# davidepi/glaze

Measured on AMD Instinct MI355X. Metric: Msamples/s + achieved HBM GB/s, Sponza 1080p, 1/2/4/8xMI355X, higher is better.
Workload: dtype f32; 1 GPU; Sponza-class synthetic atrium (262267 tris, 26 materials, 27 textures) as a .glaze V1 file (2853389 bytes) through parse, 1920x1080, path tracer depth 8, 143 steps = 17.9 spp; materials=26, textures=27, scene=Sponza-class synthetic atrium, width=1920, height=1080, depth=8, triangles=262267

## Files before the change

glaze_amd/csrc/device/path_state.h:

```cpp
#pragma once
#include <hip/hip_runtime.h>

#include "device/intersect.h"
#include "device/math.h"
#include "device/trace_wave.h"
#include "kernels.h"

namespace glz {
using namespace dev;

constexpr uint32_t kQueueShards = 8;
constexpr uint32_t kCounterStride = 32;
constexpr uint32_t kFlagUpdate = 1u;
constexpr uint32_t kFlagShadow = 2u;

struct PixelId {
  uint32_t x, y;
  bool active;
};
__device__ __forceinline__ PixelId pixel_of(const TileMap& m, uint32_t lid) {
  const uint32_t lane = lid & 63u, sub = (lid >> 6) & 63u, ltile = lid >> 12;
  const uint32_t gtile = ltile * m.world + m.rank;
  const uint32_t tx = gtile % m.tiles_x, ty = gtile / m.tiles_x;
  PixelId p;
// ... 53 lines not shown
      direction = mk3(rd.x, rd.y, rd.z);
    }
    tmin = 0.0001f;
    tmax = INFINITY;
    return true;
  }
};
__device__ __forceinline__ float4 pack_hit(const HitRecord& h) { return make_float4(h.leaf == 0xFFFFFFFFu ? INFINITY : h.t, h.u, h.v, __uint_as_float(h.leaf)); }
struct ClosestSink {
  const LaunchArgs& A;
  __device__ __forceinline__ void store(uint32_t lid, const HitRecord& h) { A.st.hit[lid] = pack_hit(h); }
};

__device__ __forceinline__ float update_mark(uint32_t ordinal) { return -(float)(ordinal < (1u << 24) ? ordinal : (1u << 24)); }
__device__ __forceinline__ void accumulate_retired(const LaunchArgs& A, uint32_t lid, vec3 c, bool add, float mark, float4 cum) {
  if (add) A.st.cumulative[lid] = make_float4(cum.x + c.x, cum.y + c.y, cum.z + c.z, mark);
  else A.st.cumulative[lid].w = mark;
}
__device__ __forceinline__ void accumulate_shaded(const LaunchArgs& A, uint32_t lid, vec3 c, bool add, bool update, float mark) {
  if (!update) return;
  if (add) {
    const float4 cum = A.st.cumulative[lid];
    A.st.cumulative[lid] = make_float4(cum.x + c.x, cum.y + c.y, cum.z + c.z, mark);
  } else {
    A.st.cumulative[lid].w = mark;
  }
}

__device__ __forceinline__ uint32_t queue_capacity(uint32_t n_local_pixels) {
  const uint32_t blocks = (n_local_pixels + kBlock - 1) / kBlock;
  return ((blocks + kQueueShards - 1) / kQueueShards) * kBlock;
}
__device__ __forceinline__ uint32_t queue_slot(uint32_t* counters, uint32_t n_local_pixels, bool push) {
  const unsigned long long m = __ballot(push);
  uint32_t slot = 0;
  if (push) {
    const uint32_t shard = ((blockIdx.x * blockDim.x + threadIdx.x) / kBlock) % kQueueShards;
    const int lane = threadIdx.x & 63;
    const int leader = __ffsll((long long)m) - 1;
    uint32_t base = 0;
    if (lane == leader) base = atomicAdd(counters + shard * kCounterStride, (uint32_t)__popcll(m));
    base = __shfl(base, leader);
    slot = shard * queue_capacity(n_local_pixels) + base + (uint32_t)__popcll(m & ((1ull << lane) - 1ull));
  }
  return slot;
}

struct ShadowSource {
  const LaunchArgs& A;
  const uint32_t* start;
  uint32_t cap;
  uint32_t lid;
  float4 contrib;
  __device__ __forceinline__ bool load(uint32_t i, vec3& o, vec3& d, float& tmin, float& tmax) {
    uint32_t shard = 0;
#pragma unroll
    for (uint32_t k = 1; k < kQueueShards; ++k) shard += i >= start[k] ? 1u : 0u;
    const uint32_t q = shard * cap + (i - start[shard]);
    const float4 so = A.st.sh_o[q], sd = A.st.sh_d[q];
    contrib = A.st.contrib[q];
    lid = __float_as_uint(sd.w);
    o = mk3(so.x, so.y, so.z);
    d = mk3(sd.x, sd.y, sd.z);
    tmin = 0.001f;
    tmax = so.w;
    return true;
  }
};
struct ShadowSink {
  const LaunchArgs& A;
  ShadowSource& src;
  __device__ __forceinline__ void store(uint32_t, const HitRecord& h) {
    const bool occluded = h.leaf != 0xFFFFFFFFu;
    const vec3 c = mk3(src.contrib.x, src.contrib.y, src.contrib.z);
    if (occluded) A.st.cumulative[src.lid].w = A.shadow_mark;
    else accumulate_retired(A, src.lid, c, true, A.shadow_mark, A.st.cumulative[src.lid]);
  }
};
__device__ __forceinline__ void clear_next_queue_set(const LaunchArgs& A) {
  if (blockIdx.x == 0 && threadIdx.x < kQueueShards) A.st.queue_count[A.shade_set * kQueueSetWords + threadIdx.x * kCounterStride] = 0;
}
}
```

glaze_amd/csrc/device/tuning.h:

```cpp
#pragma once
#ifndef GLZ_TRACE_WAVES
#define GLZ_TRACE_WAVES 6
#endif
#ifndef GLZ_TRACE_SPLIT_NUM
#define GLZ_TRACE_SPLIT_NUM 8
#endif
#ifndef GLZ_TRACE_SPLIT_DEN
#define GLZ_TRACE_SPLIT_DEN 10
#endif
#ifndef GLZ_ANY_FAR_FIRST
#define GLZ_ANY_FAR_FIRST 1
#endif
#ifndef GLZ_COUNT_ANY_FAR_FIRST
#define GLZ_COUNT_ANY_FAR_FIRST 0
#endif
#ifndef GLZ_TRACE_PREFETCH
#define GLZ_TRACE_PREFETCH 0
#endif
#ifndef GLZ_TRACE_TL_WAVES
#define GLZ_TRACE_TL_WAVES 4
#endif
#ifndef GLZ_SHADE_WAVES
#define GLZ_SHADE_WAVES 4
#endif
#ifndef GLZ_PATH_WAVES
#define GLZ_PATH_WAVES 4
#endif
#ifndef GLZ_TRACE8_WAVES
#define GLZ_TRACE8_WAVES 4
#endif
#ifndef GLZ_TRACE8_STACK
#define GLZ_TRACE8_STACK 28
#endif
#ifndef GLZ_TRACE8_PREFETCH
#define GLZ_TRACE8_PREFETCH 1
#endif
#ifndef GLZ_REFILL
#define GLZ_REFILL 10
#endif
#ifndef GLZ_REFILL_ANY
#define GLZ_REFILL_ANY GLZ_REFILL
#endif
#ifndef GLZ_LEAF_QUORUM_ANY
#define GLZ_LEAF_QUORUM_ANY 30
#endif
#ifndef GLZ_TL_REFILL
#define GLZ_TL_REFILL 16
#endif
#ifndef GLZ_LEAF_QUORUM
#define GLZ_LEAF_QUORUM 24
#endif
#ifndef GLZ_ALPHA_QUORUM
#define GLZ_ALPHA_QUORUM 12
#endif
#ifndef GLZ_TL_LEAF_QUORUM
#define GLZ_TL_LEAF_QUORUM 32
#endif
#ifndef GLZ_PATH_PREFETCH
#define GLZ_PATH_PREFETCH 1
#endif
```

glaze_amd/csrc/kernels.h:

```cpp
#pragma once
#include <hip/hip_runtime.h>
#include <stdint.h>

#include <vector>

#include "device/types.h"
#include "glaze_abi.h"
#include "device_buffer.h"
#include "reproject.h"

namespace glz {

hipError_t launch_derivatives(hipStream_t st, const float4* vertices, const uint32_t* indices, uint32_t n_tris, float4* out);

struct HierarchyInputs {
  const float4* vertices;
  const uint32_t* indices;
  const RTInstance* instances;
  const uint32_t* inst_base;
  uint32_t n_instances;
  const TransformPair* transforms;
  const RTMaterial* materials;
  uint32_t n_world;
  int builder;
  float pair_area_ratio;
  const float4* given_lo = nullptr;
  const float4* given_hi = nullptr;
  bool emit_quads = false;
  bool emit_wide8 = false;
};
constexpr int kBvhBuilderLbvh = 0, kBvhBuilderPloc = 1, kBvhBuilderSah = 2, kBvhBuilderAuto = 3, kBvhBuilderSahHost = 4;
void build_sah_host(uint32_t n, const float4* lo, const float4* hi, int2* children, int* parent);
struct HierarchyOutputs {
  DeviceBuffer<BvhNode4> nodes;
  DeviceBuffer<BvhNode8> nodes8;
  uint32_t depth8;
  BvhGrid grid;
  BvhTri* tris;
  DeviceBuffer<BvhQuad> quads;
  uint32_t depth;
  float sah;
  float bounds_lo[3], bounds_hi[3];
};
hipError_t build_hierarchy(hipStream_t st, const HierarchyInputs& in, HierarchyOutputs& out);
hipError_t launch_top_table(hipStream_t st, const BvhNode4* nodes, uint32_t n_nodes, BvhNode4* top);
hipError_t launch_shade_records(hipStream_t st, uint32_t n, const BvhTri* tris, const RTInstance* instances, const uint32_t* indices,
                                const float4* vertices, const float4* derivatives, const uint32_t* xf_identity, float4* out);
struct InstanceBoxItem {
  uint32_t transform, mesh, first, count;
};
hipError_t launch_instance_boxes(hipStream_t st, uint32_t n_items, const InstanceBoxItem* items, const float4* points, const TransformPair* xf,
                                 double* partial, uint32_t n_instances, const uint32_t* item_first, const float4* mesh_lo, const float4* mesh_hi,
                                 float4* box_lo, float4* box_hi);
hipError_t launch_alpha_records(hipStream_t st, uint32_t n, const float4* shade_tris, const RTMaterial* materials, const TexDesc* tex_desc, float4* out);

hipError_t launch_refit_leaves(hipStream_t st, const float4* vertices, const uint32_t* indices, const RTInstance* instances, const TransformPair* transforms,
                               uint32_t n_leaves, BvhQuad* quads, BvhTri* tris, float4* leaf_lo, float4* leaf_hi);
struct RefitNodes {
// ... 14 lines not shown

struct TraversalSizes {
  uint64_t n_nodes, n_nodes8, n_leaves, n_instances, grid_lanes, overflow_depth;
};
const char* traversal_offsets_exceeded(const TraversalSizes& sizes);

struct PathState {
  float4* ray_o;
  float4* ray_d;
  float4* imp[4];
  float4* hit;
  float* cone;
  uint32_t* hit_inst;
  float4* sh_o;
  float4* sh_d;
  float4* contrib;
  uint32_t* queue_count;
  float4* cumulative;
  float4* result;
  uint32_t* overflow;
  uint32_t overflow_depth;
  uint32_t* path_cost;
};

struct TileMap {
  uint32_t width, height;
  uint32_t tiles_x, tiles_y;
  uint32_t rank, world;
  uint32_t n_local_tiles;
  uint32_t n_local_pixels;
};

struct CameraConsts {
  float camera2world[16];
  float screen2camera[16];
};

struct TraceCounters {
  unsigned long long closest_rays, shadow_rays, closest_nodes, closest_tris, shadow_nodes, shadow_tris, hits, fresh;
  unsigned long long phase[12];
  unsigned long long shade_tex[4], trace_tex[4];
};

struct LaunchArgs {
  DeviceScene scene;
  PathState st;
  TileMap map;
  FrameData frame;
  CameraConsts cam;
  TraceCounters* counters;
  uint32_t do_closest, do_shadow;
  uint32_t shade_set;
  float shadow_mark;
};
constexpr uint32_t kPathMaxLaunches = 192;
struct PathBatch {
  uint32_t n;
  uint32_t tables_in_lds;
  uint32_t parity;
  uint32_t seed[kPathMaxLaunches];
  float offset[kPathMaxLaunches + 1][2];
  uint32_t base_ordinal;
};
constexpr uint32_t kTraceBlock = 256;
constexpr uint32_t kQueueSetWords = 8 * 32;

uint32_t trace_grid_blocks(uint32_t n_local_pixels, bool counting, bool two_level, bool wide8 = false);
hipError_t launch_trace(hipStream_t st, const LaunchArgs& a, uint32_t blocks, bool wide8 = false);
hipError_t launch_shade(hipStream_t st, const LaunchArgs& a);
uint32_t path_grid_blocks(uint32_t n_local_pixels, const DeviceScene& scene);
uint32_t path_resident_blocks(const DeviceScene& scene);
hipError_t launch_path(hipStream_t st, const LaunchArgs& a, const PathBatch& batch, uint32_t blocks);
hipError_t launch_finalize(hipStream_t st, const TileMap& map, float4* cumulative, float4* result, float exposure, float launches);
hipError_t launch_export(hipStream_t st, const TileMap& map, const float4* tiled, float4* frame, bool zero_first);
hipError_t launch_pack_tiles(hipStream_t st, uint32_t n_chain_pixels, uint32_t n_chains, uint32_t chain, const float4* tiled, float4* packed);
hipError_t launch_tonemap(hipStream_t st, uint32_t n_pixels, const float4* result_frame, const float* thresholds, uchar4* out);

uint32_t first_hit_grid_blocks(uint32_t n_rays);
hipError_t launch_first_hit(hipStream_t st, const LaunchArgs& a, uint32_t blocks, float4* hit, uint32_t* inst);
hipError_t launch_first_hit_attributes(hipStream_t st, const LaunchArgs& a, const float4* hit, const uint32_t* inst, float4* aov0, float4* aov1);
constexpr uint32_t kGuideCountWords = GLZ_GUIDE_MAX_BOUNCES + 2;
struct GuideLists {
  float4* o[2];
  float4* d[2];
  uint32_t* count;
};
uint32_t guide_grid_blocks(uint32_t n_rays, uint32_t first_hit_blocks);
hipError_t launch_guide_chain(hipStream_t st, const LaunchArgs& a, uint32_t blocks, uint32_t max_bounces, uint32_t last_list, float4* hit, uint32_t* inst,
                              const GuideLists& lists, float4* aov0, float4* aov1);
hipError_t launch_guide_scatter(hipStream_t st, uint32_t blocks, const GuideLists& lists, uint32_t list, uint32_t n_pixels, float* origins3, float* dirs3,
                                uint8_t* alive);
hipError_t launch_camera_rays(hipStream_t st, const LaunchArgs& a, float off_x, float off_y, float* origins3, float* dirs3);
hipError_t launch_denoise(hipStream_t st, uint32_t w, uint32_t h, const glz_denoise_params& params, const float4* result, const float4* aov0,
                          const float4* aov1, float4* ping, float4* pong, float4* out, hipEvent_t* marks = nullptr,
                          const glz_despeckle_params* despeckle = nullptr, hipEvent_t* despeckle_marks = nullptr);
hipError_t launch_despeckle(hipStream_t st, uint32_t w, uint32_t h, const glz_despeckle_params& params, float eps_albedo, const float4* result,
                            const float4* aov0, const float4* aov1, float4* ping, float4* out, hipEvent_t* despeckle_marks = nullptr);
hipError_t launch_motion(hipStream_t st, const LaunchArgs& a, const float4* hit, const uint32_t* inst, const float4* prev_o2w, const post::ProjectConstants& prev,
                         float4* motion, const float4* prev_vertices = nullptr, uint32_t first_vertex = 0, uint32_t n_vertices = 0);
hipError_t launch_reproject(hipStream_t st, uint32_t w, uint32_t h, const glz_reproject_params& params, const float4* motion, const float4* prev_color,
                            const float4* prev_aov0, const float4* prev_aov1, float4* out, hipEvent_t* marks = nullptr);
hipError_t launch_project_points(hipStream_t st, const post::ProjectConstants& C, uint32_t w, uint32_t h, const float* points3, uint32_t n, float* out3);

struct SkinArgs {
  const float4* bind;
  const uint2* joints;
  const float4* weights;
  uint32_t n;
  const float4* bones;
  uint32_t n_bones;
  int blend;
};
constexpr uint32_t kSkinLdsBones = 256;
struct MorphArgs {
  const float4* base;
  const uint32_t* counts;
  const uint2* slices;
  const float4* entries;
// ... 57 lines not shown
```

glaze_amd/csrc/kernels_render.hip:

```cpp
#include "device/path_state.h"
#include "device/shade_pixel.h"
#include "device/trace_wave.h"
#include "device/trace_wave_tl.h"
#include "launch_geometry.h"
#include "symbol_readers.h"

namespace glz {
using namespace dev;


constexpr uint32_t kShadeBlock = 256, kShadeWavesPerBlock = kShadeBlock / 64;
#ifdef GLZ_SECTION_TIMES
static __device__ unsigned long long g_shade_sections[16 * 4096];
#endif
__host__ __device__ inline bool shade_tables_fit(const DeviceScene& s) { return SceneTables(s).bytes() <= kShadeLdsTableBytes; }
__host__ __device__ inline bool shade_sky_fits(const DeviceScene& s) { return s.sky_header.marginal_cdf_count > 1u && s.sky_header.marginal_cdf_count <= kSkyLdsFloats; }
template <class T>
__device__ __forceinline__ const T* in_memory(const T* p) { return (const T*)(const __attribute__((address_space(1))) T*)p; }
template <bool COUNT, bool LOD, bool TABLES, bool SKY>
__global__ void __launch_bounds__(kShadeBlock, GLZ_SHADE_WAVES) k_shade(const LaunchArgs A) {
#ifdef GLZ_SECTION_TIMES
  unsigned long long ks[4] = {0, 0, 0, 0}, ks_last = __builtin_amdgcn_s_memtime();
#define GLZ_KS(k) do { const unsigned long long now_ = __builtin_amdgcn_s_memtime(); ks[k] += now_ - ks_last; ks_last = now_; } while (0)
#else
// ... 129 lines not shown
  {
    __syncthreads();
    float4* stage = reinterpret_cast<float4*>(s_pool);
    const uint32_t p = s_perm[threadIdx.x];
    s_bin[p] = staged.mask;
    if (staged.mask & 1u) stage[p] = staged.ro;
    if (staged.mask & 2u) stage[kShadeBlock + p] = staged.rd;
    if (staged.mask & 4u) {
#pragma unroll
      for (int q = 0; q < 4; ++q) stage[(2u + q) * kShadeBlock + p] = staged.im[q];
    }
    __syncthreads();
    const LaunchArgs& A3 = *(const LaunchArgs*)reread_kernarg();
    const uint32_t m = s_bin[threadIdx.x], at = blockIdx.x * kShadeBlock + threadIdx.x;
    if (m & 1u) A3.st.ray_o[at] = stage[threadIdx.x];
    if (m & 2u) A3.st.ray_d[at] = stage[kShadeBlock + threadIdx.x];
    if (m & 4u) {
#pragma unroll
      for (int q = 0; q < 4; ++q) A3.st.imp[q][at] = stage[(2u + q) * kShadeBlock + threadIdx.x];
    }
  }
  if (COUNT) flush_tex_tallies(A.counters->shade_tex, tex_tally);
#ifdef GLZ_SECTION_TIMES
  if (!COUNT) {
    GLZ_KS(3);
    unsigned long long v[10] = {ks[0], ks[1], ks[2], staged.sec[0], staged.sec[1], staged.sec[2], staged.sec[3], staged.sec[4], staged.sec[5], ks[3]};
    const uint32_t w = blockIdx.x * kShadeWavesPerBlock + (threadIdx.x >> 6);
#pragma unroll
    for (int k = 0; k < 10; ++k) {
      unsigned int lo = (unsigned int)v[k], hi = (unsigned int)(v[k] >> 32);
      for (int off = 32; off > 0; off >>= 1) {
        const unsigned int lo2 = __shfl_xor(lo, off), hi2 = __shfl_xor(hi, off);
        const unsigned long long a = ((unsigned long long)hi << 32) | lo, b = ((unsigned long long)hi2 << 32) | lo2;
        if (b > a) { lo = lo2; hi = hi2; }
      }
      if ((threadIdx.x & 63u) == 0u && w < 4096u) g_shade_sections[16u * w + k] += ((unsigned long long)hi << 32) | lo;
    }
    if ((threadIdx.x & 63u) == 0u && w < 4096u) g_shade_sections[16u * w + 15u] += 1ull;
  }
#endif
}

template <bool COUNT, int ALPHA>
__global__ void __launch_bounds__(kBlock, GLZ_TRACE_WAVES) k_trace(const LaunchArgs A) {
  __shared__ int s_stack[kLdsStack * kBlock];
  __shared__ alignas(1024) int s_aux[kAuxPerBlock];
  __shared__ uint4 s_top[kBvhTopNodes * 4];
  static_assert(kBvhTopNodes * 4 <= kBlock, "stage_top copies one 16-byte piece per thread");
  GLZ_WAVE_STAMP(0);
  stage_top(A.scene, s_top);
  int* aux = wave_aux(s_aux, threadIdx.x >> 6);
  int* links = wave_links(s_aux, threadIdx.x >> 6);
  clear_next_queue_set(A);
  unsigned long long tex_tally[4] = {0ull, 0ull, 0ull, 0ull};
  DeviceScene counted_scene;
  if (COUNT) {
    counted_scene = A.scene;
    counted_scene.tex_counter = tex_tally;
  }
  const DeviceScene& TS = COUNT ? counted_scene : A.scene;
  uint32_t split_closest = A.do_closest, split_shadow = A.do_shadow, split_wave_c = wave_index(), split_waves_c = wave_count(), split_wave_s = 0, split_waves_s = 0;
  bool split = false;
  if (!COUNT && A.do_closest && A.do_shadow) {
    const uint32_t* counts0 = A.st.queue_count + (A.shade_set ^ 1u) * kQueueSetWords;
    uint32_t n_sh = 0;
#pragma unroll
    for (uint32_t k = 0; k < kQueueShards; ++k) n_sh += counts0[k * kCounterStride];
    const uint32_t gc = (A.map.n_local_pixels + 63u) / 64u, gs = (n_sh + 63u) / 64u, nw = wave_count();
    if (gc + gs > nw && gs > 0u) {
      split = true;
      uint32_t ws = (uint32_t)(((unsigned long long)nw * gs * GLZ_TRACE_SPLIT_NUM) / ((unsigned long long)gc * GLZ_TRACE_SPLIT_DEN + (unsigned long long)gs * GLZ_TRACE_SPLIT_NUM));
      ws = ws < 1u ? 1u : (ws > nw - 1u ? nw - 1u : ws);
      const uint32_t w = wave_index();
      const uint32_t s_before = (uint32_t)(((unsigned long long)w * ws) / nw), s_after = (uint32_t)(((unsigned long long)(w + 1u) * ws) / nw);
      const bool is_shadow = s_after > s_before;
      split_closest = is_shadow ? 0u : 1u;
      split_shadow = is_shadow ? 1u : 0u;
      split_wave_c = w - s_before;
      split_waves_c = nw - ws;
      split_wave_s = s_before;
      split_waves_s = ws;
    }
  }
  if (split_closest) {
    TraceTally tally;
    ClosestSource src{A, A.frame, tally, 0u};
    ClosestSink sink{A};
    trace_wave<false, COUNT, false, GLZ_TRACE_PREFETCH != 0, false, ALPHA>(TS, src, sink, &s_stack[threadIdx.x], aux, links, (LdsNodePtr)s_top, A.st.overflow, A.st.overflow_depth, A.map.n_local_pixels, split_wave_c,
                                                         split_waves_c, tally);
    if (COUNT) flush_counters(A.counters, false, tally);
  }
  GLZ_WAVE_STAMP(1);
  if (split_shadow) {
    const uint32_t* counts = A.st.queue_count + (A.shade_set ^ 1u) * kQueueSetWords;
    uint32_t start[kQueueShards + 1];
    start[0] = 0;
#pragma unroll
    for (uint32_t k = 0; k < kQueueShards; ++k) start[k + 1] = start[k] + counts[k * kCounterStride];
    TraceTally tally;
    ShadowSource src{A, start, queue_capacity(A.map.n_local_pixels), 0u, make_float4(0.0f, 0.0f, 0.0f, 0.0f)};
    ShadowSink sink{A, src};
    uint32_t n_waves = wave_count();
    const uint32_t closest_groups = A.do_closest ? (A.map.n_local_pixels + 63u) / 64u : 0u;
    uint32_t wave = (wave_index() + n_waves - closest_groups % n_waves) % n_waves;
    if (split) { wave = split_wave_s; n_waves = split_waves_s; }
    trace_wave<true, COUNT, false, GLZ_TRACE_PREFETCH != 0, false, ALPHA>(TS, src, sink, &s_stack[threadIdx.x], aux, links, (LdsNodePtr)s_top, A.st.overflow, A.st.overflow_depth, start[kQueueShards], wave, n_waves, tally);
    if (COUNT) flush_counters(A.counters, true, tally);
  }
  if (COUNT) flush_tex_tallies(A.counters->trace_tex, tex_tally);
  GLZ_WAVE_STAMP(2);
}

__global__ void __launch_bounds__(kBlock, GLZ_TRACE8_WAVES) k_trace8(const LaunchArgs A) {
  __shared__ int s_stack[kLdsStack8 * kBlock];
  __shared__ alignas(1024) int s_aux[kAuxPerBlock];
  int* aux = wave_aux(s_aux, threadIdx.x >> 6);
  int* links = wave_links(s_aux, threadIdx.x >> 6);
  clear_next_queue_set(A);
  if (A.do_closest) {
    TraceTally tally;
    ClosestSource src{A, A.frame, tally, 0u};
    ClosestSink sink{A};
    trace_wave<false, false, false, GLZ_TRACE8_PREFETCH != 0, true>(A.scene, src, sink, &s_stack[threadIdx.x], aux, links, (LdsNodePtr) nullptr, A.st.overflow, A.st.overflow_depth,
                                                                    A.map.n_local_pixels, wave_index(), wave_count(), tally);
  }
  if (A.do_shadow) {
    const uint32_t* counts = A.st.queue_count + (A.shade_set ^ 1u) * kQueueSetWords;
    uint32_t start[kQueueShards + 1];
    start[0] = 0;
#pragma unroll
    for (uint32_t k = 0; k < kQueueShards; ++k) start[k + 1] = start[k] + counts[k * kCounterStride];
    TraceTally tally;
    ShadowSource src{A, start, queue_capacity(A.map.n_local_pixels), 0u, make_float4(0.0f, 0.0f, 0.0f, 0.0f)};
    ShadowSink sink{A, src};
    const uint32_t n_waves = wave_count();
    const uint32_t closest_groups = A.do_closest ? (A.map.n_local_pixels + 63u) / 64u : 0u;
    const uint32_t wave = (wave_index() + n_waves - closest_groups % n_waves) % n_waves;
    trace_wave<true, false, false, GLZ_TRACE8_PREFETCH != 0, true>(A.scene, src, sink, &s_stack[threadIdx.x], aux, links, (LdsNodePtr) nullptr, A.st.overflow, A.st.overflow_depth,
                                                                   start[kQueueShards], wave, n_waves, tally);
  }
}

struct ClosestSinkTl {
  const LaunchArgs& A;
  __device__ __forceinline__ void store(uint32_t lid, const HitRecord& h) {
    A.st.hit[lid] = pack_hit(h);
    A.st.hit_inst[lid] = h.inst;
  }
};
template <bool COUNT>
__global__ void __launch_bounds__(kBlock, GLZ_TRACE_TL_WAVES) k_trace_tl(const LaunchArgs A) {
  __shared__ int s_stack[kLdsStack * kBlock];
  __shared__ alignas(1024) int s_aux[kAuxPerBlock];
  __shared__ float s_top_ray[9 * kBlock];
  __shared__ uint4 s_top[kTlLdsTop ? kBvhTopNodes * 4 : 1];
  if (kTlLdsTop) stage_top(A.scene, s_top);
  int* aux = wave_aux(s_aux, threadIdx.x >> 6);
  int* links = wave_links(s_aux, threadIdx.x >> 6);
  clear_next_queue_set(A);
// ... 146 lines not shown
```

glaze_amd/csrc/renderer.cpp:

```cpp
#include "renderer.h"

#include <algorithm>
#include <cmath>
#include <cstdlib>
#include <cstring>

namespace glz {

namespace {
inline bool timed_launch(uint64_t i , uint64_t stride) {
  const uint64_t group = (i - 1) / stride;
  uint32_t x = (uint32_t)group * 747796405u + 2891336453u;
  x = ((x >> ((x >> 28) + 4u)) ^ x) * 277803737u;
  x ^= x >> 22;
  return (i - 1) % stride == x % stride;
}
}
uint64_t Renderer::event_stride() const {
  uint64_t pixels = 0;
  for (const auto& c : chains_) pixels += c->map.n_local_pixels;
  return pixels >= (1u << 20) ? 4u : 16u;
}

Renderer* Renderer::create(Instance* inst, std::shared_ptr<Scene> scene, uint32_t w, uint32_t h, Error& err) {
  std::unique_ptr<Renderer> r(new Renderer());
  r->inst_ = inst;
  if (!hip_ok(hipSetDevice(inst->device), "hipSetDevice", err)) return nullptr;
  if (!scene) {
    SceneData empty;
    empty.camera = default_camera();
    empty.meta = default_meta();
    scene.reset(Scene::create(inst, std::move(empty), err));
    if (!scene) return nullptr;
  }
  r->scene_ = scene;
  if (w == 0 || h == 0) {
    err.fail(GLZ_E_ARG, "resolution must be non-zero");
    return nullptr;
  }
  r->w_ = w;
  r->h_ = h;
  r->cfg_.camera = scene->data.camera;
  r->cfg_.exposure = scene->data.meta.exposure;
  host::push_constants(r->cfg_.camera, w, h, r->cfg_.cam.camera2world, r->cfg_.cam.screen2camera);
  if (!r->allocate(err)) return nullptr;
  return r.release();
}

void Renderer::release_chains() {
  for (auto& c : chains_) {
    if (c->stream) (void)hipStreamSynchronize(c->stream);
    for (auto& s : c->pending_events)
      for (auto& e : s.e) (void)hipEventDestroy(e);
    for (auto& s : c->free_events)
      for (auto& e : s.e) (void)hipEventDestroy(e);
    if (c->own_stream && c->stream) (void)hipStreamDestroy(c->stream);
  }
  chains_.clear();
// ... 3 lines not shown
  group_.release();
  if (inst_) (void)hipSetDevice(inst_->device);
  release_chains();
}

uint32_t Renderer::chains_for(uint32_t w, uint32_t h, uint32_t rank, uint32_t world, uint32_t wanted) {
  const TileMap m = make_tile_map(w, h, rank, world);
  const uint32_t local_tiles = m.n_local_tiles;
  const uint64_t pixels = m.n_local_pixels;
  uint32_t want = wanted;
  if (want == 0) want = pixels >= 1000000u ? 1u : (pixels >= 400000u ? 2u : 3u);
  if (want > local_tiles) want = local_tiles;
  return want ? want : 1u;
}
uint32_t Renderer::pick_chains() const { return path_mode_ ? 1u : chains_for(w_, h_, rank_, world_, cfg_.chains_wanted); }

bool Renderer::allocate(Error& err) {
  release_chains();
  {
    const uint64_t pixels = make_tile_map(w_, h_, rank_, world_).n_local_pixels;
    bool fits = false;
    if (cfg_.launch_mode == 0 && pixels > 0 && pixels <= (1u << 22) && scene_->dev.two_level == 0) {
      const uint32_t blocks = (uint32_t)((pixels / 64 + kTraceBlock / 64 - 1) / (kTraceBlock / 64));
      const uint32_t resident = path_resident_blocks(scene_->dev);
      fits = resident >= blocks && (scene_->info.n_world_triangles < 4096 || (uint64_t)blocks * 5u <= (uint64_t)resident * 4u);
    }
    path_mode_ = scene_->dev.two_level == 0 && (cfg_.launch_mode == 2 || fits);
    wide8_ = scene_->dev.two_level == 0 && scene_->dev.bvh_nodes8 != nullptr && cfg_.node_width == 8;
  }
  const uint32_t S = pick_chains();
  const uint32_t od = scene_->accel().stack_overflow_depth;
  for (uint32_t s = 0; s < S; ++s) {
    std::unique_ptr<Chain> c(new Chain());
    if (s == 0) {
      c->stream = inst_->stream;
    } else {
      if (!hip_ok(hipStreamCreateWithFlags(&c->stream, hipStreamNonBlocking), "hipStreamCreate", err)) return false;
      c->own_stream = true;
    }
    const TileMap& m = c->map = make_chain_map(w_, h_, rank_, world_, s, S);
    const size_t n = m.n_local_pixels;
    const size_t n_queue = (((n + 255) / 256 + 7) / 8) * 256 * 8;
    DeviceBuffer<float4>* bufs[] = {&c->ray_o, &c->ray_d, &c->imp[0], &c->imp[1], &c->imp[2], &c->imp[3], &c->hit, &c->sh_o, &c->sh_d, &c->contrib,
                                    &c->cumulative, &c->result};
    for (auto* b : bufs)
      if (!hip_ok(b->alloc((b == &c->sh_o || b == &c->sh_d || b == &c->contrib) ? n_queue : n), "alloc path state", err)) return false;
    if (!hip_ok(c->cone.alloc(n), "alloc path state", err)) return false;
    if (!hip_ok(c->hit_inst.alloc(n), "alloc path state", err)) return false;
    c->grid = trace_grid_blocks(m.n_local_pixels, false, scene_->dev.two_level != 0);
    c->grid_counting = trace_grid_blocks(m.n_local_pixels, true, scene_->dev.two_level != 0);
    c->grid8 = wide8_ ? trace_grid_blocks(m.n_local_pixels, false, false, true) : 0u;
    c->grid_path = path_mode_ ? path_grid_blocks(m.n_local_pixels, scene_->dev) : 0u;
    if (!hip_ok(c->overflow.alloc((size_t)std::max(std::max(std::max(c->grid, c->grid_counting), c->grid_path), c->grid8) * kTraceBlock * od), "alloc traversal spill", err)) return false;
    if (!hip_ok(c->queue_count.alloc(2 * kQueueSetWords), "alloc queue counters", err)) return false;
    if (!hip_ok(c->path_cost.alloc(8 + n / 64 + 1), "alloc path costs", err)) return false;
    if (!hip_ok(hipMemsetAsync(c->path_cost.ptr, 0, sizeof(uint32_t) * (8 + n / 64 + 1), c->stream), "clear path costs", err)) return false;
    chains_.push_back(std::move(c));
  }
  if (!hip_ok(frame_tmp_.alloc((size_t)w_ * h_), "alloc frame", err)) return false;
  if (!hip_ok(rgba8_.alloc((size_t)w_ * h_), "alloc rgba8", err)) return false;
  if (!oetf_thresholds_.ptr) {
    float thr[256];
    host::srgb8_thresholds(thr);
    if (!hip_ok(oetf_thresholds_.upload(thr, 256, chains_[0]->stream), "upload OETF thresholds", err)) return false;
    if (!hip_ok(hipStreamSynchronize(chains_[0]->stream), "upload OETF thresholds", err)) return false;
  }
  if (!hip_ok(counters_.alloc(1), "alloc counters", err)) return false;
  request_new_frame_ = true;
  return true;
}

bool Renderer::reset_buffers(Error& err) {
  for (auto& c : chains_)
    if (!hip_ok(hipStreamSynchronize(c->stream), "reset", err)) return false;
  for (auto& cp : chains_) {
    Chain& c = *cp;
    const size_t bytes = sizeof(float4) * (size_t)c.map.n_local_pixels;
    DeviceBuffer<float4>* zero[] = {&c.ray_o, &c.ray_d, &c.imp[0], &c.imp[1], &c.imp[2], &c.imp[3], &c.cumulative, &c.result, &c.contrib};
    for (auto* b : zero)
      if (bytes && !hip_ok(hipMemsetAsync(b->ptr, 0, bytes, c.stream), "clear path state", err)) return false;
    if (!hip_ok(hipMemsetAsync(c.queue_count.ptr, 0, sizeof(uint32_t) * 2 * kQueueSetWords, c.stream), "clear queue counters", err)) return false;
    c.shadow_pending = false;
    c.trace_ms = c.shade_ms = c.flush_ms = c.path_ms = 0;
    for (auto& s : c.pending_events) c.free_events.push_back(s);
    c.pending_events.clear();
  }
  if (!hip_ok(hipMemsetAsync(counters_.ptr, 0, sizeof(TraceCounters), chains_[0]->stream), "clear counters", err)) return false;
  if (chains_.size() > 1 && !hip_ok(hipStreamSynchronize(chains_[0]->stream), "clear counters", err)) return false;
  sched_.rewind();
  rng_.reseed(cfg_.seed);
  launches_ = 0;
  accum_launches_ = 0;
  resolve_pending_ = false;
  request_new_frame_ = false;
  return true;
}

void Renderer::fill_args(const Chain& c, LaunchArgs& a) const {
  a.scene = scene_->dev;
  a.st.ray_o = c.ray_o.ptr;
  a.st.ray_d = c.ray_d.ptr;
  for (int q = 0; q < 4; ++q) a.st.imp[q] = c.imp[q].ptr;
  a.st.hit = c.hit.ptr;
  a.st.cone = c.cone.ptr;
  a.st.hit_inst = c.hit_inst.ptr;
  a.st.sh_o = c.sh_o.ptr;
  a.st.sh_d = c.sh_d.ptr;
  a.st.contrib = c.contrib.ptr;
  a.st.queue_count = c.queue_count.ptr;
  a.st.cumulative = c.cumulative.ptr;
  a.st.result = c.result.ptr;
  a.st.overflow = c.overflow.ptr;
  a.st.overflow_depth = scene_->accel().stack_overflow_depth;
  a.st.path_cost = c.path_cost.ptr;
  a.map = c.map;
  a.cam = cfg_.cam;
  a.counters = cfg_.counting ? counters_.ptr : nullptr;
  a.do_closest = a.do_shadow = 0;
  a.shade_set = c.pending_set ^ 1u;
  a.shadow_mark = c.pending_mark;
}

void Renderer::resolve_events(Chain& c) {
  for (auto& s : c.pending_events) {
    float a = 0, b = 0;
    (void)hipEventElapsedTime(&a, s.e[0], s.e[1]);
    if (s.kind == 1) {
      c.flush_ms += a;
    } else if (s.kind == 2) {
      c.path_ms += a;
    } else {
      (void)hipEventElapsedTime(&b, s.e[1], s.e[2]);
      const double weight = (double)s.weight;
      c.trace_ms += a * weight;
      c.shade_ms += b * weight;
    }
    c.free_events.push_back(s);
  }
  c.pending_events.clear();
}

bool Renderer::acquire_events(Chain& c, EventSet& ev, Error& err) {
  if (c.free_events.empty()) {
    if (c.pending_events.size() >= 64) {
      if (!hip_ok(hipEventSynchronize(last_event(c.pending_events.back())), "hipEventSynchronize", err)) return false;
      resolve_events(c);
    }
    if (c.free_events.empty()) {
      EventSet fresh{};
      for (auto& e : fresh.e)
        if (!hip_ok(hipEventCreateWithFlags(&e, hipEventDisableSystemFence), "hipEventCreate", err)) return false;
      c.free_events.push_back(fresh);
    }
  }
  ev = c.free_events.back();
  c.free_events.pop_back();
  return true;
}

struct Renderer::Timed {
  Chain& c;
  EventSet ev{};
  bool on = false;
  bool begin(Renderer& r, bool timed, int kind, uint32_t weight, Error& err) {
    on = timed;
    if (!on) return true;
    if (!r.acquire_events(c, ev, err)) return false;
    ev.kind = kind;
    ev.weight = weight;
    (void)hipEventRecord(ev.e[0], c.stream);
    return true;
  }
  void mark() {
// ... 626 lines not shown
```

glaze_amd/csrc/renderer.h:

```cpp
#pragma once
#include <algorithm>
#include <cstdlib>
#include <initializer_list>
#include <memory>
#include <vector>

#include "device_group.h"
#include "host_math.h"
#include "kernels.h"
#include "post_stage.h"
#include "scene.h"
#include "tile_map.h"

namespace glz {

class Renderer {
 public:
  static Renderer* create(Instance* inst, std::shared_ptr<Scene> scene , uint32_t w, uint32_t h, Error& err);
  ~Renderer();

  bool set_integrator(int integrator, Error& err);
  bool set_exposure(float e, Error& err);
  bool update_camera(const glz_camera& c, Error& err);
  bool change_resolution(uint32_t w, uint32_t h, Error& err);
  bool change_scene(std::shared_ptr<Scene> scene, Error& err);
  bool update_materials_and_lights(const glz_material* m, uint32_t nm, const glz_light* l, uint32_t nl, const glz_texture* t, uint32_t nt, Error& err);
  bool refresh_binded_textures(const glz_texture* t, uint32_t nt, Error& err);
  bool update_transforms(const glz_transform* t, uint32_t n, Error& err);
  bool update_vertices(const glz_vertex* v, uint32_t first, uint32_t n, int mode, Error& err);
  int add_skin(const glz_skin& skin, Error& err);
  bool remove_skin(int id, Error& err);
  bool set_skin_blend(int id, int blend, Error& err);
  bool pose_skins(const glz_pose* poses, uint32_t n, int mode, Error& err);
  int add_morph(const glz_morph& morph, Error& err);
  bool remove_morph(int id, Error& err);
  bool animate(const glz_animation& anim, int mode, Error& err);
  int add_skeleton(const glz_skeleton& skeleton, Error& err);
  bool remove_skeleton(int id, Error& err);
  int add_clip(const glz_clip& clip, Error& err);
  bool remove_clip(int id, Error& err);
  bool play(const glz_play* plays, uint32_t n, int mode, Error& err);
  int add_normals(const glz_normals& set, Error& err);
  bool remove_normals(int id, Error& err);
  bool read_vertices(uint32_t first, uint32_t n, glz_vertex* out, Error& err);
  bool geometry_update_info(glz_geometry_update_info& out, Error& err);
  bool wait_idle(Error& err);
  uint32_t steps_per_sample() const { return cfg_.integrator == GLZ_DIRECT ? 1u : cfg_.pt_steps; }

  bool draw(size_t spp, void (*cb)(void*), void* user, uint8_t* rgba8_out, Error& err);
  bool restart();
  bool step(uint32_t n, Error& err);
  bool read_rgba8(uint8_t* out, Error& err);
  bool read_frame(bool result, float* out, Error& err);
  PostStage& post() { return post_; }
  bool read_denoised(float* rgba32f, uint8_t* rgba8, Error& err) { return read_post(true, rgba32f, rgba8, err); }
  bool read_despeckled(float* rgba32f, uint8_t* rgba8, Error& err) { return read_post(false, rgba32f, rgba8, err); }
  bool time_post(float ms[GLZ_POST_TIMING_SLOTS], Error& err);

  bool set_texture_lod(int mode, Error& err);
  bool set_seed(uint64_t s);
  bool set_depth(uint32_t d, Error& err);
  bool set_partition(uint32_t rank, uint32_t world, Error& err);
  bool set_devices(const int* devices, int n, Error& err);
  uint32_t device_count() const { return 1u + (uint32_t)group_.size(); }
  const Scene* device_scene(int i) const { return i == 0 ? scene_.get() : group_.scene(i); }
  bool set_chains(uint32_t n, Error& err);
  bool set_launch_mode(int mode, Error& err);
// ... 16 lines not shown
  Instance* instance() const { return inst_; }
  Scene* scene() const { return scene_.get(); }
  uint32_t width() const { return w_; }
  uint32_t height() const { return h_; }
  const CameraConsts& camera_consts() const { return cfg_.cam; }
  bool perspective() const { return cfg_.camera.type == GLZ_CAMERA_PERSPECTIVE; }
  struct HostCopy {
    void* out;
    const void* dev;
    size_t bytes;
  };
  bool to_host(std::initializer_list<HostCopy> copies, const char* what, Error& err) const;
  bool frame_to_host(const float4* frame, void* out, const char* what, Error& err) const { return to_host({{out, frame, sizeof(float4) * (size_t)w_ * h_}}, what, err); }

  void take_settings(const Renderer& root) { cfg_ = root.cfg_; }
  bool set_partition_local(uint32_t rank, uint32_t world, Error& err);
  bool settle(Error& err);
  bool gather(bool result, float4* dst, Error& err, bool zero_first = true);
  struct PackedTiles {
    const TileMap& map;
    const float4* data;
  };
  PackedTiles packed_tiles(uint32_t chain, bool result) const { return {chains_[chain]->map, result ? chains_[chain]->result.ptr : chains_[chain]->cumulative.ptr}; }

 private:
  Renderer() = default;
  bool allocate(Error& err);
  bool reset_buffers(Error& err);
  bool one_launch(Error& err);
  bool launch_constants_common(FrameData& fd, Error& err);
  bool path_batch(uint32_t n, Error& err);
  bool run_launches(uint32_t n, Error& err);
  bool use_path() const { return path_mode_ && !cfg_.counting && chains_.size() == 1 && chains_[0]->grid_path != 0; }
  template <class A> bool resize(A apply, Error& err);
  template <class U> bool update_scene(U update, Error& err);
  bool rgba8_to_host(const float4* frame, uint8_t* out, const char* what, const char* what_sync, Error& err);

  Instance* inst_ = nullptr;
  std::shared_ptr<Scene> scene_;
  uint32_t w_ = 0, h_ = 0;
  struct Settings {
    int integrator = GLZ_PATH_TRACE;
    uint32_t pt_steps = 6;
    int lod_mode = 0;
    float exposure = 1.0f;
    glz_camera camera{};
    CameraConsts cam{};
    uint64_t seed = 0;
    uint32_t chains_wanted = 0;
    int launch_mode = getenv("GLAZE_LAUNCH_MODE") ? atoi(getenv("GLAZE_LAUNCH_MODE")) : 0;
    int node_width = getenv("GLAZE_NODE_WIDTH") ? atoi(getenv("GLAZE_NODE_WIDTH")) : 0;
    bool counting = false;
    bool profile_kernels = true;
  } cfg_;
  host::SeedStream rng_;
  host::WorkScheduler sched_;
  bool request_new_frame_ = true;
  uint32_t rank_ = 0, world_ = 1;
  bool path_mode_ = false;
  bool wide8_ = false;

  struct EventSet {
    hipEvent_t e[4];
    int kind;
    uint32_t weight;
  };
  static hipEvent_t last_event(const EventSet& s) { return s.e[s.kind ? 1 : 2]; }
  struct Timed;
  uint64_t event_stride() const;
  struct Chain {
    TileMap map{};
    hipStream_t stream = nullptr;
    bool own_stream = false;
    DeviceBuffer<float4> ray_o, ray_d, imp[4], hit, sh_o, sh_d, contrib, cumulative, result;
    DeviceBuffer<float> cone;
    DeviceBuffer<uint32_t> hit_inst;
    DeviceBuffer<uint32_t> overflow, queue_count, path_cost;
    uint32_t path_batches = 0;
    uint32_t grid = 0, grid_counting = 0;
    uint32_t grid8 = 0;
    uint32_t grid_path = 0;
    bool shadow_pending = false;
    uint32_t pending_set = 0;
    float pending_mark = 0.0f;
    std::vector<EventSet> pending_events;
    std::vector<EventSet> free_events;
    double trace_ms = 0, shade_ms = 0, flush_ms = 0, path_ms = 0;
  };
  std::vector<std::unique_ptr<Chain>> chains_;
  uint32_t pick_chains() const;
  uint32_t trace_grid(const Chain& c) const { return cfg_.counting ? c.grid_counting : (wide8() ? c.grid8 : c.grid); }
  void release_chains();
  bool flush_shadows(Chain& c, Error& err);
  bool resolve(Error& err);
  float update_mark() const { return -(float)std::min<uint64_t>(accum_launches_, 1u << 24); }
  bool acquire_events(Chain& c, EventSet& ev, Error& err);
  void resolve_events(Chain& c);
  void fill_args(const Chain& c, LaunchArgs& a) const;

  DeviceGroup group_{*this};
  bool wait_idle_local(const char* what, Error& err);
  bool step_local(uint32_t n, Error& err);

  bool frame_is_here(const char* who, Error& err) const;
  bool read_post(bool filter, float* rgba32f, uint8_t* rgba8, Error& err, hipEvent_t* marks = nullptr);
  PostStage post_{*this};
// ... 12 lines not shown
```

Baseline: 3263 Msamples/s.

## Add chunked shadow-ray work pool to split trace and retune split ratio

Factors the closest/shadow wave split into a reusable plan. It adds an optional dynamic pool: waves that finish early grab chunks of the shadow queue through an atomic head counter, which is cleared each launch. By default the pool fraction is zero, so only the static split runs. The default share of waves given to shadow rays is lowered from 8/10 to 6/10 weighting. Extra readfirstlane calls keep the control values wave-uniform. The pool adds an atomic per chunk and more control flow in exchange for better tail balancing when it is enabled.

```diff
diff --git a/glaze_amd/csrc/device/path_state.h b/glaze_amd/csrc/device/path_state.h
--- a/glaze_amd/csrc/device/path_state.h
+++ b/glaze_amd/csrc/device/path_state.h
@@ -129,7 +129,9 @@
   uint32_t cap;
   uint32_t lid;
   float4 contrib;
+  uint32_t base = 0u;
   __device__ __forceinline__ bool load(uint32_t i, vec3& o, vec3& d, float& tmin, float& tmax) {
+    i += base;
     uint32_t shard = 0;
 #pragma unroll
     for (uint32_t k = 1; k < kQueueShards; ++k) shard += i >= start[k] ? 1u : 0u;
@@ -157,4 +159,7 @@
 __device__ __forceinline__ void clear_next_queue_set(const LaunchArgs& A) {
   if (blockIdx.x == 0 && threadIdx.x < kQueueShards) A.st.queue_count[A.shade_set * kQueueSetWords + threadIdx.x * kCounterStride] = 0;
 }
+__device__ __forceinline__ void clear_next_pool_head(const LaunchArgs& A) {
+  if (blockIdx.x == 0 && threadIdx.x == kQueueShards) A.st.queue_count[pool_head_word(A.shade_set)] = 0;
 }
+}
diff --git a/glaze_amd/csrc/device/trace_split.h b/glaze_amd/csrc/device/trace_split.h
--- /dev/null
+++ b/glaze_amd/csrc/device/trace_split.h
@@ -0,0 +1,55 @@
+#pragma once
+#include <hip/hip_runtime.h>
+#include <stdint.h>
+
+namespace glz {
+
+struct TraceSplitTuning {
+  uint32_t static_num, static_den;
+  uint32_t pool_num, pool_den;
+  uint32_t chunk_groups;
+};
+
+struct TraceSplit {
+  uint32_t split;
+  uint32_t ws;
+  uint32_t n_static;
+  uint32_t chunk_groups;
+  uint32_t n_chunks;
+};
+
+__host__ __device__ inline TraceSplit trace_split_plan(uint32_t gc, uint32_t n_sh, uint32_t nw, const TraceSplitTuning& t) {
+  TraceSplit p{0u, 0u, 0u, 0u, 0u};
+  const uint32_t gs = (n_sh + 63u) / 64u;
+  if (nw < 2u || gs == 0u || (unsigned long long)gc + gs <= nw) return p;
+  p.split = 1u;
+  const unsigned long long s_part = (unsigned long long)gs * t.static_num, c_part = (unsigned long long)gc * t.static_den;
+  const uint32_t ws = s_part + c_part ? (uint32_t)(((unsigned long long)nw * s_part) / (c_part + s_part)) : 0u;
+  p.ws = ws < 1u ? 1u : (ws > nw - 1u ? nw - 1u : ws);
+  uint32_t pool_groups = t.pool_den ? (uint32_t)(((unsigned long long)gs * t.pool_num) / t.pool_den) : 0u;
+  pool_groups = pool_groups > gs ? gs : pool_groups;
+  p.n_static = pool_groups ? (gs - pool_groups) * 64u : n_sh;
+  p.chunk_groups = t.chunk_groups < 1u ? 1u : t.chunk_groups;
+  p.n_chunks = (pool_groups + p.chunk_groups - 1u) / p.chunk_groups;
+  return p;
+}
+
+__host__ __device__ inline uint32_t trace_split_chunk_first(const TraceSplit& p, uint32_t c) { return p.n_static + c * p.chunk_groups * 64u; }
+__host__ __device__ inline uint32_t trace_split_chunk_rays(const TraceSplit& p, uint32_t c, uint32_t n_sh) {
+  const uint32_t first = trace_split_chunk_first(p, c), left = n_sh - first;
+  return left < p.chunk_groups * 64u ? left : p.chunk_groups * 64u;
+}
+
+struct TraceWaveRole {
+  uint32_t is_shadow, index, count;
+};
+__host__ __device__ inline TraceWaveRole trace_split_role(const TraceSplit& p, uint32_t w, uint32_t nw) {
+  const uint32_t s_before = (uint32_t)(((unsigned long long)w * p.ws) / nw), s_after = (uint32_t)(((unsigned long long)(w + 1u) * p.ws) / nw);
+  TraceWaveRole r;
+  r.is_shadow = s_after > s_before ? 1u : 0u;
+  r.index = r.is_shadow ? s_before : w - s_before;
+  r.count = r.is_shadow ? p.ws : nw - p.ws;
+  return r;
+}
+
+}
diff --git a/glaze_amd/csrc/device/tuning.h b/glaze_amd/csrc/device/tuning.h
--- a/glaze_amd/csrc/device/tuning.h
+++ b/glaze_amd/csrc/device/tuning.h
@@ -3,10 +3,19 @@
 #define GLZ_TRACE_WAVES 6
 #endif
 #ifndef GLZ_TRACE_SPLIT_NUM
-#define GLZ_TRACE_SPLIT_NUM 8
+#define GLZ_TRACE_SPLIT_NUM 6
 #endif
 #ifndef GLZ_TRACE_SPLIT_DEN
 #define GLZ_TRACE_SPLIT_DEN 10
+#endif
+#ifndef GLZ_TRACE_POOL_NUM
+#define GLZ_TRACE_POOL_NUM 0
+#endif
+#ifndef GLZ_TRACE_POOL_DEN
+#define GLZ_TRACE_POOL_DEN 1
+#endif
+#ifndef GLZ_TRACE_POOL_CHUNK
+#define GLZ_TRACE_POOL_CHUNK 2
 #endif
 #ifndef GLZ_ANY_FAR_FIRST
 #define GLZ_ANY_FAR_FIRST 1
diff --git a/glaze_amd/csrc/kernels.h b/glaze_amd/csrc/kernels.h
--- a/glaze_amd/csrc/kernels.h
+++ b/glaze_amd/csrc/kernels.h
@@ -4,6 +4,7 @@
 
 #include <vector>
 
+#include "device/trace_split.h"
 #include "device/types.h"
 #include "glaze_abi.h"
 #include "device_buffer.h"
@@ -124,6 +125,7 @@
   uint32_t do_closest, do_shadow;
   uint32_t shade_set;
   float shadow_mark;
+  TraceSplitTuning split;
 };
 constexpr uint32_t kPathMaxLaunches = 192;
 struct PathBatch {
@@ -136,6 +138,9 @@
 };
 constexpr uint32_t kTraceBlock = 256;
 constexpr uint32_t kQueueSetWords = 8 * 32;
+constexpr uint32_t kPoolHeadStride = 32;
+constexpr uint32_t kQueueCountWords = 2 * kQueueSetWords + 2 * kPoolHeadStride;
+constexpr uint32_t pool_head_word(uint32_t set) { return 2 * kQueueSetWords + set * kPoolHeadStride; }
 
 uint32_t trace_grid_blocks(uint32_t n_local_pixels, bool counting, bool two_level, bool wide8 = false);
 hipError_t launch_trace(hipStream_t st, const LaunchArgs& a, uint32_t blocks, bool wide8 = false);
diff --git a/glaze_amd/csrc/kernels_render.hip b/glaze_amd/csrc/kernels_render.hip
--- a/glaze_amd/csrc/kernels_render.hip
+++ b/glaze_amd/csrc/kernels_render.hip
@@ -205,6 +205,7 @@
   int* aux = wave_aux(s_aux, threadIdx.x >> 6);
   int* links = wave_links(s_aux, threadIdx.x >> 6);
   clear_next_queue_set(A);
+  clear_next_pool_head(A);
   unsigned long long tex_tally[4] = {0ull, 0ull, 0ull, 0ull};
   DeviceScene counted_scene;
   if (COUNT) {
@@ -212,52 +213,66 @@
     counted_scene.tex_counter = tex_tally;
   }
   const DeviceScene& TS = COUNT ? counted_scene : A.scene;
-  uint32_t split_closest = A.do_closest, split_shadow = A.do_shadow, split_wave_c = wave_index(), split_waves_c = wave_count(), split_wave_s = 0, split_waves_s = 0;
-  bool split = false;
+  const auto uniform = [](uint32_t v) { return (uint32_t)__builtin_amdgcn_readfirstlane((int)v); };
+  const uint32_t* counts = A.st.queue_count + (A.shade_set ^ 1u) * kQueueSetWords;
+  const uint32_t closest_groups = A.do_closest ? (A.map.n_local_pixels + 63u) / 64u : 0u;
+  uint32_t split_closest = A.do_closest, split_wave_c = wave_index(), split_waves_c = wave_count();
+  uint32_t sh_trip = A.do_shadow, sh_total = 0xFFFFFFFFu , sh_waves = wave_count(), sh_wave = (wave_index() + sh_waves - closest_groups % sh_waves) % sh_waves, sh_base = 0u;
+  TraceSplit plan{0u, 0u, 0u, 0u, 0u};
   if (!COUNT && A.do_closest && A.do_shadow) {
-    const uint32_t* counts0 = A.st.queue_count + (A.shade_set ^ 1u) * kQueueSetWords;
     uint32_t n_sh = 0;
 #pragma unroll
-    for (uint32_t k = 0; k < kQueueShards; ++k) n_sh += counts0[k * kCounterStride];
-    const uint32_t gc = (A.map.n_local_pixels + 63u) / 64u, gs = (n_sh + 63u) / 64u, nw = wave_count();
-    if (gc + gs > nw && gs > 0u) {
-      split = true;
-      uint32_t ws = (uint32_t)(((unsigned long long)nw * gs * GLZ_TRACE_SPLIT_NUM) / ((unsigned long long)gc * GLZ_TRACE_SPLIT_DEN + (unsigned long long)gs * GLZ_TRACE_SPLIT_NUM));
-      ws = ws < 1u ? 1u : (ws > nw - 1u ? nw - 1u : ws);
-      const uint32_t w = wave_index();
-      const uint32_t s_before = (uint32_t)(((unsigned long long)w * ws) / nw), s_after = (uint32_t)(((unsigned long long)(w + 1u) * ws) / nw);
-      const bool is_shadow = s_after > s_before;
-      split_closest = is_shadow ? 0u : 1u;
-      split_shadow = is_shadow ? 1u : 0u;
-      split_wave_c = w - s_before;
-      split_waves_c = nw - ws;
-      split_wave_s = s_before;
-      split_waves_s = ws;
-    }
-  }
+    for (uint32_t k = 0; k < kQueueShards; ++k) n_sh += counts[k * kCounterStride];
+    plan = trace_split_plan(closest_groups, uniform(n_sh), wave_count(), A.split);
+    if (plan.split) {
+      const TraceWaveRole role = trace_split_role(plan, wave_index(), wave_count());
+      split_closest = role.is_shadow ? 0u : 1u;
+      split_wave_c = role.index;
+      split_waves_c = wave_count() - plan.ws;
+      sh_trip = role.is_shadow;
+      sh_total = plan.n_static;
+      sh_wave = role.index;
+      sh_waves = plan.ws;
+    }
+  }
+  const TraceSplit pool{plan.split, 0u, uniform(plan.n_static), uniform(plan.chunk_groups), uniform(plan.n_chunks)};
+  split_closest = uniform(split_closest);
   if (split_closest) {
     TraceTally tally;
     ClosestSource src{A, A.frame, tally, 0u};
     ClosestSink sink{A};
-    trace_wave<false, COUNT, false, GLZ_TRACE_PREFETCH != 0, false, ALPHA>(TS, src, sink, &s_stack[threadIdx.x], aux, links, (LdsNodePtr)s_top, A.st.overflow, A.st.overflow_depth, A.map.n_local_pixels, split_wave_c,
-                                                         split_waves_c, tally);
+    trace_wave<false, COUNT, false, GLZ_TRACE_PREFETCH != 0, false, ALPHA>(TS, src, sink, &s_stack[threadIdx.x], aux, links, (LdsNodePtr)s_top, A.st.overflow, A.st.overflow_depth, A.map.n_local_pixels, uniform(split_wave_c),
+                                                         uniform(split_waves_c), tally);
     if (COUNT) flush_counters(A.counters, false, tally);
   }
   GLZ_WAVE_STAMP(1);
-  if (split_shadow) {
-    const uint32_t* counts = A.st.queue_count + (A.shade_set ^ 1u) * kQueueSetWords;
+  if (A.do_shadow) {
     uint32_t start[kQueueShards + 1];
     start[0] = 0;
 #pragma unroll
-    for (uint32_t k = 0; k < kQueueShards; ++k) start[k + 1] = start[k] + counts[k * kCounterStride];
+    for (uint32_t k = 0; k < kQueueShards; ++k) start[k + 1] = uniform(start[k] + counts[k * kCounterStride]);
+    const uint32_t n_sh = start[kQueueShards];
+    if (!pool.split) sh_total = n_sh;
     TraceTally tally;
     ShadowSource src{A, start, queue_capacity(A.map.n_local_pixels), 0u, make_float4(0.0f, 0.0f, 0.0f, 0.0f)};
     ShadowSink sink{A, src};
-    uint32_t n_waves = wave_count();
-    const uint32_t closest_groups = A.do_closest ? (A.map.n_local_pixels + 63u) / 64u : 0u;
-    uint32_t wave = (wave_index() + n_waves - closest_groups % n_waves) % n_waves;
-    if (split) { wave = split_wave_s; n_waves = split_waves_s; }
-    trace_wave<true, COUNT, false, GLZ_TRACE_PREFETCH != 0, false, ALPHA>(TS, src, sink, &s_stack[threadIdx.x], aux, links, (LdsNodePtr)s_top, A.st.overflow, A.st.overflow_depth, start[kQueueShards], wave, n_waves, tally);
+    sh_trip = uniform(sh_trip); sh_total = uniform(sh_total); sh_wave = uniform(sh_wave); sh_waves = uniform(sh_waves);
+    for (;;) {
+      if (!sh_trip) {
+        if (pool.n_chunks == 0u) break;
+        uint32_t c = 0u;
+        if ((threadIdx.x & 63u) == 0u) c = atomicAdd(A.st.queue_count + pool_head_word(A.shade_set ^ 1u), 1u);
+        c = uniform(c);
+        if (c >= pool.n_chunks) break;
+        sh_base = uniform(trace_split_chunk_first(pool, c));
+        sh_total = uniform(trace_split_chunk_rays(pool, c, n_sh));
+        sh_wave = 0u;
+        sh_waves = 1u;
+      }
+      sh_trip = 0u;
+      src.base = sh_base;
+      trace_wave<true, COUNT, false, GLZ_TRACE_PREFETCH != 0, false, ALPHA>(TS, src, sink, &s_stack[threadIdx.x], aux, links, (LdsNodePtr)s_top, A.st.overflow, A.st.overflow_depth, sh_total, sh_wave, sh_waves, tally);
+    }
     if (COUNT) flush_counters(A.counters, true, tally);
   }
   if (COUNT) flush_tex_tallies(A.counters->trace_tex, tex_tally);
diff --git a/glaze_amd/csrc/renderer.cpp b/glaze_amd/csrc/renderer.cpp
--- a/glaze_amd/csrc/renderer.cpp
+++ b/glaze_amd/csrc/renderer.cpp
@@ -2,8 +2,11 @@
 
 #include <algorithm>
 #include <cmath>
+#include <cstdio>
 #include <cstdlib>
 #include <cstring>
+
+#include "device/tuning.h"
 
 namespace glz {
 
@@ -113,7 +116,7 @@
     c->grid8 = wide8_ ? trace_grid_blocks(m.n_local_pixels, false, false, true) : 0u;
     c->grid_path = path_mode_ ? path_grid_blocks(m.n_local_pixels, scene_->dev) : 0u;
     if (!hip_ok(c->overflow.alloc((size_t)std::max(std::max(std::max(c->grid, c->grid_counting), c->grid_path), c->grid8) * kTraceBlock * od), "alloc traversal spill", err)) return false;
-    if (!hip_ok(c->queue_count.alloc(2 * kQueueSetWords), "alloc queue counters", err)) return false;
+    if (!hip_ok(c->queue_count.alloc(kQueueCountWords), "alloc queue counters", err)) return false;
     if (!hip_ok(c->path_cost.alloc(8 + n / 64 + 1), "alloc path costs", err)) return false;
     if (!hip_ok(hipMemsetAsync(c->path_cost.ptr, 0, sizeof(uint32_t) * (8 + n / 64 + 1), c->stream), "clear path costs", err)) return false;
     chains_.push_back(std::move(c));
@@ -140,7 +143,7 @@
     DeviceBuffer<float4>* zero[] = {&c.ray_o, &c.ray_d, &c.imp[0], &c.imp[1], &c.imp[2], &c.imp[3], &c.cumulative, &c.result, &c.contrib};
     for (auto* b : zero)
       if (bytes && !hip_ok(hipMemsetAsync(b->ptr, 0, bytes, c.stream), "clear path state", err)) return false;
-    if (!hip_ok(hipMemsetAsync(c.queue_count.ptr, 0, sizeof(uint32_t) * 2 * kQueueSetWords, c.stream), "clear queue counters", err)) return false;
+    if (!hip_ok(hipMemsetAsync(c.queue_count.ptr, 0, sizeof(uint32_t) * kQueueCountWords, c.stream), "clear queue counters", err)) return false;
     c.shadow_pending = false;
     c.trace_ms = c.shade_ms = c.flush_ms = c.path_ms = 0;
     for (auto& s : c.pending_events) c.free_events.push_back(s);
@@ -180,6 +183,17 @@
   a.do_closest = a.do_shadow = 0;
   a.shade_set = c.pending_set ^ 1u;
   a.shadow_mark = c.pending_mark;
+  a.split = cfg_.trace_split;
+}
+
+TraceSplitTuning trace_split_from_env() {
+  TraceSplitTuning t{GLZ_TRACE_SPLIT_NUM, GLZ_TRACE_SPLIT_DEN, GLZ_TRACE_POOL_NUM, GLZ_TRACE_POOL_DEN, GLZ_TRACE_POOL_CHUNK};
+  unsigned v[5];
+  const char* s = getenv("GLAZE_TRACE_SPLIT");
+  if (s && sscanf(s, "%u/%u,%u/%u,%u", &v[0], &v[1], &v[2], &v[3], &v[4]) == 5 && v[0] >= 1 && v[1] >= 1 && v[3] >= 1 && v[2] <= v[3] && v[4] >= 1 &&
+      v[0] <= 65535 && v[1] <= 65535 && v[3] <= 65535 && v[4] <= 65535)
+    t = TraceSplitTuning{v[0], v[1], v[2], v[3], v[4]};
+  return t;
 }
 
 void Renderer::resolve_events(Chain& c) {
diff --git a/glaze_amd/csrc/renderer.h b/glaze_amd/csrc/renderer.h
--- a/glaze_amd/csrc/renderer.h
+++ b/glaze_amd/csrc/renderer.h
@@ -13,6 +13,8 @@
 #include "tile_map.h"
 
 namespace glz {
+
+TraceSplitTuning trace_split_from_env();
 
 class Renderer {
  public:
@@ -135,6 +137,7 @@
     int node_width = getenv("GLAZE_NODE_WIDTH") ? atoi(getenv("GLAZE_NODE_WIDTH")) : 0;
     bool counting = false;
     bool profile_kernels = true;
+    TraceSplitTuning trace_split = trace_split_from_env();
   } cfg_;
   host::SeedStream rng_;
   host::WorkScheduler sched_;
```

Result: faster. 3327 Msamples/s (median of 6 runs) (+2.0%).
